# ericyinyzy/VQAttack

Measured on AMD Instinct MI355X. Metric: adversarial_vqa_examples_per_sec, higher is better.
Workload: dtype f32; 1 GPU; vlmo_base VQAttack image PGD (BASELINE configs[1]): batch 64 per GPU, 40 PGD steps, 384x384 images, questions of 6..14 real tokens ([CLS] + n words + [SEP], n ~ U{4..12} seeded) padded to 40 (the all-padding columns are not run through the encoder), eps 0.125 step 0.01 L-inf clip [-1,1], random start, sanity_checks on, black-box scoring + ASR gather; batch_per_gpu=64, pgd_steps=40, image_size=384, text_len=40, substitutable_words=0

## Files before the change

### include/vqattack_hip.h

```cpp
#ifndef VQATTACK_HIP_H
#define VQATTACK_HIP_H

#include <stddef.h>
#include <stdint.h>

#ifdef __cplusplus
extern "C" {
#endif

typedef void* vqa_stream_t;

#define VQA_OK 0
#define VQA_ERR_NULL (-1)
#define VQA_ERR_SHAPE (-2)
#define VQA_ERR_ALIGN (-3)

#define VQA_CLIP 1u
#define VQA_CHECK_RANGE 2u
#define VQA_FLAG_RANGE 1
#define VQA_FLAG_BAD_LABEL 2
#define VQA_FLAG_DEGENERATE 4

int vqa_abi_version(void);
const char* vqa_error_string(int code);
// ... 40 lines not shown

int vqa_l1_fgm(const float* x, const float* g, const float* amax, const float* ties, float* out, int batch,
               size_t n_per_sample, float eps_iter, float cmin, float cmax, unsigned mode, int* flag,
               vqa_stream_t stream);

int vqa_scale_per_sample(const float* t, const float* stat, const float* stat2, float* out, int batch,
                         size_t n_per_sample, float eps, int kind, int* flag, vqa_stream_t stream);

int vqa_neg_cos_partials(void);
int vqa_neg_cos_rows(const float* a, const float* b, float* ga, float* partial, const uint8_t* row_mask,
                     long mask_period, long rows0, long rows1, int D, long a_stride0, long a_stride1,
                     long b_stride0, long b_stride1, long g_stride0, long g_stride1, float gscale,
                     float cos_eps, float* loss_out, int accumulate, vqa_stream_t stream);

int vqa_neg_cos_max_layers(void);
int vqa_neg_cos_rows_multi(const float* const* a, const float* const* b, float* const* ga, int n_layers,
                           float* partial, const uint8_t* row_mask, long mask_period, long rows0, long rows1, int D,
                           long a_stride0, long a_stride1, long b_stride0, long b_stride1, long g_stride0,
                           long g_stride1, float gscale, float cos_eps, float* loss_out, int accumulate,
                           vqa_stream_t stream);

int vqa_sum_partials(const float* partial, int count, float* dst, int accumulate, float scale,
                     vqa_stream_t stream);

int vqa_ce_max_label_sets(void);
long vqa_ce_scratch_floats(int K, long groups);
int vqa_ce_rows(const float* logits, long row_stride, const int64_t* labels, int K, long rows, int V,
                long ignore_index, long rows_per_group, float* scratch, float* grad, float* row_loss, float gscale,
                float* loss_out, int accumulate, int* flag, unsigned char* row_state, vqa_stream_t stream);

int vqa_gather_rows(const float* src, const int64_t* idx, float* dst, int B, int L, int K, int D,
                    vqa_stream_t stream);

int vqa_cand_dir_sim(const float* word, const float* pos, const float* type, const float* gamma,
                     const float* beta, float ln_eps, const float* e_ori, const float* grad,
                     const int32_t* cand, float* out, int n_cand, int L, int K, int D, vqa_stream_t stream);

int vqa_embed_tokens(const float* word, const float* pos, const float* type, const float* gamma, const float* beta,
                     float ln_eps, const int32_t* triples, int n, float* dst, int D, vqa_stream_t stream);

int vqa_greedy_accept(const int32_t* cand, const int32_t* order, const int32_t* seg, int B, int L,
                      const int64_t* ori_ids, int64_t* cur_ids, int32_t* new_id, int32_t* acc_rank, const float* table,
                      int V, int E, float threshold, vqa_stream_t stream);

int vqa_attn_fwd(const float* q, const float* k, const float* v, const float* bias, float* o, float* lse, float* scores,
                 int B, int H, int Sq, int Sk, const long* strides, const long* bias_strides, float scale,
                 const int* key_hole, int nsplit, float* split_ws, vqa_stream_t stream);
long vqa_attn_scores_floats(int B, int H, int Sq, int Sk);
long vqa_attn_split_ws_floats(int B, int H, int Sq, int Sk, int nsplit);

int vqa_attn_bwd(const float* q, const float* k, const float* v, const float* bias, const float* o, const float* go,
                 const float* lse, const float* scores, float* delta, float* dq, float* dk, float* dv, float* ds_ws, int B,
                 int H, int Sq, int Sk, const long* strides, const long* bias_strides, const long* grad_strides,
                 float scale, int nsplit, float* split_ws, vqa_stream_t stream);
long vqa_attn_bwd_ws_floats(int B, int H, int Sq, int Sk);

int vqa_resize_bicubic_h_u8(const uint8_t* src, int h, int w_in, int c, const int32_t* kk, const int32_t* bounds,
                            int ksize, int w_out, uint8_t* dst, vqa_stream_t stream);
int vqa_resize_bicubic_v_normalize(const uint8_t* src, int h_in, int w, int c, const int32_t* kk,
                                   const int32_t* bounds, int ksize, int h_out, float mean, float stdv, float* dst,
                                   vqa_stream_t stream);

int vqa_ln_fwd(const float* x, const float* r0, const float* r1, const float* rscale, float* x_out,
               const float* gamma0, const float* beta0, const float* gamma1, const float* beta1, float* y0, float* y1,
               float* mean, float* rstd, long rows, int D, long period, long split, float eps, vqa_stream_t stream);
int vqa_ln_bwd(const float* dy0, const float* dy1, const float* x, const float* mean, const float* rstd,
               const float* gamma0, const float* gamma1, const float* g_a, const float* g_inj, const float* rscale,
               float* dx, float* dr0, float* dr1, long rows, int D, long period, long split, vqa_stream_t stream);
int vqa_ln_bwd_post(const float* dy_a, const float* dy_b, const float* g_inj, const float* s, const float* rstd,
                    const float* gamma, float* ds, long rows, int D, vqa_stream_t stream);
int vqa_gelu_fwd(const float* h, float* a, size_t n, vqa_stream_t stream);
int vqa_gelu_bwd(const float* h, const float* da, float* dh, size_t n, vqa_stream_t stream);

size_t vqa_gemm_packed_bytes(int K, int N);
int vqa_gemm_pack_b(const float* w, long ldw, int trans, void* packed, int K, int N, vqa_stream_t stream);
int vqa_gemm_bf16x6(const float* A, long lda, const void* packed, const float* bias, float* C, long ldc, long M, int N,
                    int K, vqa_stream_t stream);

#define VQA_GEMM_TILE_256X128 0
#define VQA_GEMM_TILE_128X256 1
int vqa_gemm_bf16x6_tile(const float* A, long lda, const void* packed, const float* bias, float* C, long ldc, long M,
                         int N, int K, int tile, vqa_stream_t stream);

int vqa_gemm_bf16x6_half(const float* A, long lda, const void* packed, const float* bias, float* C, long ldc, long M,
                         int N, int K, vqa_stream_t stream);
int vqa_gemm_bf16x6_tail(const float* A, long lda, const void* packed, const float* bias, float* C, long ldc, long M,
                         int N, int K, int tile, long m_split, vqa_stream_t stream);

size_t vqa_gemm_small_ws_bytes(long M, int N, int ksplit);
int vqa_gemm_bf16x6_small(const float* A, long lda, const void* packed, const float* bias, float* C, long ldc, long M,
                          int N, int K, int ksplit, void* ws, vqa_stream_t stream);

#define VQA_GEMM_EPI_NONE 0
#define VQA_GEMM_EPI_GELU 1
#define VQA_GEMM_EPI_GELU_GRAD 2
int vqa_gemm_bf16x6_epi(const float* A, long lda, const void* packed, const float* bias, float* C, long ldc, long M,
                        int N, int K, int tile, int epilogue, float* aux, long ldaux, vqa_stream_t stream);

#define VQA_GEMM_MAX_GROUPS 4
int vqa_gemm_bf16x6_grouped(const float* const* A, const long* lda, const void* const* packed, const float* const* bias,
                            float* const* C, const long* ldc, float* const* aux, const long* ldaux, const long* M,
                            int n_groups, int N, int K, int epilogue, vqa_stream_t stream);

long vqa_gemm_lse_ws_floats(long M, int N);
int vqa_gemm_bf16x6_lse(const float* A, long lda, const void* packed, const float* bias, long M, int N, int K,
                        int n_valid, const int64_t* targets, long ignore_index, float* ws, float* row_loss, float* lse,
                        int* flag, int tile, vqa_stream_t stream);

#ifdef __cplusplus
}
#endif
#endif
```

### vqattack_amd/_hip.py

```python
import ctypes
import os
import threading

import torch

_HERE = os.path.dirname(os.path.abspath(__file__))
LIB_PATH = os.path.join(_HERE, "lib", "libvqattack_hip.so")
TUNING_LIB_PATH = os.path.join(_HERE, "lib", "libvqattack_hip_tuning.so")

VQA_CLIP = 1
VQA_CHECK_RANGE = 2
VQA_FLAG_RANGE = 1
VQA_FLAG_BAD_LABEL = 2
VQA_FLAG_DEGENERATE = 4
ABI_VERSION = 4

_c_float_p = ctypes.c_void_p
_sz = ctypes.c_size_t
_f = ctypes.c_float
_i = ctypes.c_int
_u = ctypes.c_uint
_l = ctypes.c_long
_p = ctypes.c_void_p

SIGNATURES = {
    "vqa_abi_version": (_i, []),
    "vqa_error_string": (ctypes.c_char_p, [_i]),
    "vqa_linf_init": (_i, [_p, _p, _p, _sz, _f, _f, _f, _u, _p, _p]),
    "vqa_linf_fgm": (_i, [_p, _p, _p, _sz, _f, _f, _f, _u, _p, _p]),
    "vqa_linf_step": (_i, [_p, _p, _p, _p, _sz, _f, _f, _f, _f, _u, _p, _p]),
    "vqa_linf_project": (_i, [_p, _p, _p, _sz, _f, _f, _f, _u, _p]),
    "vqa_clip_eta_linf": (_i, [_p, _p, _sz, _f, _p]),
    "vqa_optimize_linear_linf": (_i, [_p, _p, _sz, _f, _p]),
    "vqa_zero_out_clipped_grads": (_i, [_p, _p, _p, _sz, _f, _f, _p]),
    "vqa_reduce_ws_bytes": (_sz, [_i, _sz]),
    "vqa_sumsq_per_sample": (_i, [_p, _p, _p, _i, _sz, _p, _p]),
    "vqa_absmax_ties_per_sample": (_i, [_p, _p, _p, _i, _sz, _p, _p]),
    "vqa_l2_fgm": (_i, [_p, _p, _p, _p, _i, _sz, _f, _f, _f, _u, _p, _p]),
    "vqa_l2_project": (_i, [_p, _p, _p, _p, _i, _sz, _f, _f, _f, _u, _p]),
    "vqa_l1_fgm": (_i, [_p, _p, _p, _p, _p, _i, _sz, _f, _f, _f, _u, _p, _p]),
    "vqa_scale_per_sample": (_i, [_p, _p, _p, _p, _i, _sz, _f, _i, _p, _p]),
    "vqa_neg_cos_partials": (_i, []),
    "vqa_neg_cos_rows": (_i, [_p, _p, _p, _p, _p, _l, _l, _l, _i, _l, _l, _l, _l, _l, _l, _f, _f, _p, _i, _p]),
    "vqa_neg_cos_max_layers": (_i, []),
    "vqa_neg_cos_rows_multi": (_i, [_p, _p, _p, _i, _p, _p, _l, _l, _l, _i, _l, _l, _l, _l, _l, _l, _f, _f, _p, _i, _p]),
    "vqa_sum_partials": (_i, [_p, _i, _p, _i, _f, _p]),
    "vqa_ce_max_label_sets": (_i, []),
    "vqa_ce_scratch_floats": (_l, [_i, _l]),
    "vqa_ce_rows": (_i, [_p, _l, _p, _i, _l, _i, _l, _l, _p, _p, _p, _f, _p, _i, _p, _p, _p]),
    "vqa_gather_rows": (_i, [_p, _p, _p, _i, _i, _i, _i, _p]),
    "vqa_cand_dir_sim": (_i, [_p, _p, _p, _p, _p, _f, _p, _p, _p, _p, _i, _i, _i, _i, _p]),
    "vqa_embed_tokens": (_i, [_p, _p, _p, _p, _p, _f, _p, _i, _p, _i, _p]),
    "vqa_greedy_accept": (_i, [_p, _p, _p, _i, _i, _p, _p, _p, _p, _p, _i, _i, _f, _p]),
    "vqa_attn_fwd": (_i, [_p, _p, _p, _p, _p, _p, _p, _i, _i, _i, _i, _p, _p, _f, _p, _i, _p, _p]),
    "vqa_attn_split_ws_floats": (_l, [_i, _i, _i, _i, _i]),
    "vqa_attn_scores_floats": (_l, [_i, _i, _i, _i]),
    "vqa_attn_bwd": (_i, [_p, _p, _p, _p, _p, _p, _p, _p, _p, _p, _p, _p, _p, _i, _i, _i, _i, _p, _p, _p, _f, _i, _p, _p]),
    "vqa_attn_bwd_ws_floats": (_l, [_i, _i, _i, _i]),
    "vqa_ln_fwd": (_i, [_p] * 13 + [_l, _i, _l, _l, _f, _p]),
    "vqa_ln_bwd": (_i, [_p] * 13 + [_l, _i, _l, _l, _p]),
    "vqa_ln_bwd_post": (_i, [_p] * 7 + [_l, _i, _p]),
    "vqa_gelu_fwd": (_i, [_p, _p, _sz, _p]),
    "vqa_gelu_bwd": (_i, [_p, _p, _p, _sz, _p]),
    "vqa_resize_bicubic_h_u8": (_i, [_p, _i, _i, _i, _p, _p, _i, _i, _p, _p]),
    "vqa_resize_bicubic_v_normalize": (_i, [_p, _i, _i, _i, _p, _p, _i, _i, _f, _f, _p, _p]),
    "vqa_gemm_packed_bytes": (_sz, [_i, _i]),
    "vqa_gemm_pack_b": (_i, [_p, _l, _i, _p, _i, _i, _p]),
    "vqa_gemm_bf16x6": (_i, [_p, _l, _p, _p, _p, _l, _l, _i, _i, _p]),
    "vqa_gemm_bf16x6_tile": (_i, [_p, _l, _p, _p, _p, _l, _l, _i, _i, _i, _p]),
    "vqa_gemm_bf16x6_half": (_i, [_p, _l, _p, _p, _p, _l, _l, _i, _i, _p]),
    "vqa_gemm_bf16x6_tail": (_i, [_p, _l, _p, _p, _p, _l, _l, _i, _i, _i, _l, _p]),
    "vqa_gemm_small_ws_bytes": (_sz, [_l, _i, _i]),
    "vqa_gemm_bf16x6_small": (_i, [_p, _l, _p, _p, _p, _l, _l, _i, _i, _i, _p, _p]),
    "vqa_gemm_bf16x6_epi": (_i, [_p, _l, _p, _p, _p, _l, _l, _i, _i, _i, _i, _p, _l, _p]),
    "vqa_gemm_bf16x6_grouped": (_i, [_p, _p, _p, _p, _p, _p, _p, _p, _p, _i, _i, _i, _i, _p]),
    "vqa_gemm_lse_ws_floats": (_l, [_l, _i]),
    "vqa_gemm_bf16x6_lse": (_i, [_p, _l, _p, _p, _l, _i, _i, _i, _p, _l, _p, _p, _p, _p, _i, _p]),
}

_lib = None
_lock = threading.Lock()


class HipExtensionError(RuntimeError):
    pass


def load_library(path=None):
    tuning = os.environ.get("VQA_TUNING_LIB", "") not in ("", "0")
    if path is None:
        path = TUNING_LIB_PATH if tuning else LIB_PATH
    if not os.path.exists(path):
        raise HipExtensionError(
            "HIP kernel library not found at {} -- build it with `python -m vqattack_amd.build` "
            "(or __graft_entry__.build()); vqattack_amd has no CPU or eager fallback".format(path))
    if tuning and path == TUNING_LIB_PATH:
        from . import build as _build
        if _build._stale(path):
            raise HipExtensionError("{} is older than vqattack_amd/csrc: rebuild it with `python -m vqattack_amd.build "
                                    "--tuning`".format(path))
    lib = ctypes.CDLL(path)
    for name, (res, args) in SIGNATURES.items():
        fn = getattr(lib, name)
        fn.restype = res
        fn.argtypes = args
    if lib.vqa_abi_version() != ABI_VERSION:
        raise HipExtensionError("{} implements C ABI version {}, this package binds version {}: rebuild it with "
                                "`python -m vqattack_amd.build --force`".format(path, lib.vqa_abi_version(), ABI_VERSION))
    options = [item for item in os.environ.get("VQA_OPTIONS", "").split(",") if item]
    if options:
        if not hasattr(lib, "vqa_set_option"):
            raise HipExtensionError("VQA_OPTIONS needs the tuning build: `python -m vqattack_amd.build --tuning` and "
                                    "VQA_TUNING_LIB=1 ({} has no vqa_set_option)".format(path))
        lib.vqa_set_option.restype, lib.vqa_set_option.argtypes = _i, [_i, _i]
        for item in options:
            opt, val = item.split("=")
            if lib.vqa_set_option(int(opt), int(val)) != 0:
                raise HipExtensionError("bad VQA_OPTIONS entry '{}'".format(item))
    return lib


def lib():
    global _lib
    if _lib is None:
        with _lock:
            if _lib is None:
                _lib = load_library()
    return _lib


def set_option(option, value):
    handle = lib()
    if not hasattr(handle, "vqa_set_option"):
        return False
    handle.vqa_set_option.restype, handle.vqa_set_option.argtypes = _i, [_i, _i]
    if handle.vqa_set_option(int(option), int(value)) != 0:
        raise HipExtensionError("vqa_set_option({}, {}) rejected".format(option, value))
    return True


def check(code, what):
    if code != 0:
        msg = lib().vqa_error_string(code)
        raise HipExtensionError("{} failed: {} ({})".format(what, msg.decode() if msg else "?", code))


def stream_for(t):
    return ctypes.c_void_p(torch.cuda.current_stream(t.device).cuda_stream)


def dev_f32(t, name, contiguous=True):
    if not isinstance(t, torch.Tensor):
# ... 21 lines not shown
```

### vqattack_amd/csrc/gemm.hip

```cpp
#include "common.hpp"
#include "gelu.hpp"

namespace vqa {

typedef __bf16 bf16x8 __attribute__((ext_vector_type(8)));
typedef __bf16 bf16x2 __attribute__((ext_vector_type(2)));
typedef float f32x4 __attribute__((ext_vector_type(4)));

constexpr int kGemmBM = 256, kGemmBN = 128, kGemmBK = 32;
constexpr int kGemmThreads = 512;
constexpr int kGemmMT = kGemmBM / 16, kGemmNT = kGemmBN / 16;
constexpr int kTileBytes = 64 * 16;
constexpr int kGemmABytes = kGemmMT * 3 * kTileBytes;
constexpr int kGemmBBytes = kGemmNT * 3 * kTileBytes;
constexpr int kGemmStage = kGemmABytes + kGemmBBytes;
constexpr int kGemmBPieces = kGemmBBytes / 16 / kGemmThreads;
constexpr int kWideLoadPair = 12;

__device__ __forceinline__ void split2(f32x2 a, bf16x2& h0, bf16x2& h1, bf16x2& h2) {
  h0 = __builtin_convertvector(a, bf16x2);
  f32x2 r = a - __builtin_convertvector(h0, f32x2);
  r.x = __builtin_isfinite(r.x) ? r.x : 0.0f;
  r.y = __builtin_isfinite(r.y) ? r.y : 0.0f;
  h1 = __builtin_convertvector(r, bf16x2);
// ... 692 lines not shown
  long r = m0 + wave * 16 + (lane & 15);
  r = r < g.M ? r : g.M - 1;
  const float* arow = g.A + r * g.lda + 8 * (lane >> 4);
  const bf16x8* bsrc = g.B + static_cast<size_t>(nb) * kWideNT * 3 * 64;
  const size_t bstep = static_cast<size_t>(nt16) * 3 * 64;

  f32x4 ra[2];
  auto load = [&](int kt) {
    ra[0] = *reinterpret_cast<const f32x4*>(arow + kt * kGemmBK);
    ra[1] = *reinterpret_cast<const f32x4*>(arow + kt * kGemmBK + 4);
  };
  char* const bwave = smem + kWideABytes + wave_u * kTileBytes;
  auto load_b = [&](int kt, int s, int p) {
    stage_b16(bsrc + kt * bstep + p * kGemmThreads + tid, bwave + s * kWideStage + p * kGemmThreads * 16);
  };
  auto store = [&](int s) {
    char* base = smem + s * kWideStage;
    bf16x8 p0, p1, p2;
    split8(ra[0], ra[1], p0, p1, p2);
    bf16x8* dst = reinterpret_cast<bf16x8*>(base) + wave * 3 * 64 + lane;
    dst[0] = p0;
    dst[64] = p1;
    dst[128] = p2;
  };

  f32x4 acc[4][4];
#pragma unroll
  for (int i = 0; i < 4; ++i)
#pragma unroll
    for (int j = 0; j < 4; ++j) acc[i][j] = f32x4{0.0f, 0.0f, 0.0f, 0.0f};

  load(0);
#pragma unroll
  for (int p = 0; p < kWideBPieces; ++p) load_b(0, 0, p);
  store(0);
  stage_b_wait();
  __syncthreads();
  for (int kt = 0; kt < nk; ++kt) {
    const int cur = kt & 1;
    const int nxt = kt + 1 < nk ? kt + 1 : kt;
    load(nxt);
    const bf16x8* sa = reinterpret_cast<const bf16x8*>(smem + cur * kWideStage) + wm * 4 * 3 * 64 + lane;
    const bf16x8* sb = reinterpret_cast<const bf16x8*>(smem + cur * kWideStage + kWideABytes) + wn * 4 * 3 * 64 + lane;
    bf16x8 fa[3][4], fb[3][4];
#pragma unroll
    for (int i = 0; i < 4; ++i)
#pragma unroll
      for (int p = 0; p < 3; ++p) {
        fa[p][i] = sa[(i * 3 + p) * 64];
        fb[p][i] = sb[(i * 3 + p) * 64];
      }
    constexpr int kPa[6] = {2, 1, 0, 1, 0, 0}, kPb[6] = {0, 1, 2, 0, 1, 0};
#pragma unroll
    for (int t = 0; t < 6; ++t) {
      if (t == 3) store(cur ^ 1);
#pragma unroll
      for (int i = 0; i < 4; ++i)
#pragma unroll
        for (int j = 0; j < 4; ++j) {
          acc[i][j] = __builtin_amdgcn_mfma_f32_16x16x32_bf16(fb[kPb[t]][j], fa[kPa[t]][i], acc[i][j], 0, 0, 0);
          if ((t * 16 + i * 4 + j + 1) % kWideLoadPair == 0 && (t * 16 + i * 4 + j + 1) / kWideLoadPair <= kWideBPieces / 2) {
            const int pair = (t * 16 + i * 4 + j + 1) / kWideLoadPair - 1;
            load_b(nxt, cur ^ 1, 2 * pair);
            load_b(nxt, cur ^ 1, 2 * pair + 1);
          }
        }
    }
#pragma unroll
    for (int n = 0; n < (2 + kWideBPieces) / 2; ++n) {
      __builtin_amdgcn_sched_group_barrier(0x020, 2, 0);
      __builtin_amdgcn_sched_group_barrier(0x008, kWideLoadPair, 0);
    }
    stage_b_wait();
    __syncthreads();
  }

  if constexpr (EPI == VQA_GEMM_EPI_NONE) {
    gemm_store(acc, g, m0 + wm * 64, n0 + wn * 64, lane);
  } else {
    gemm_epilogue<EPI>(acc, g, m0 + wm * 64, n0 + wn * 64, lane);
  }
}

constexpr int kSmallBM = 64;
constexpr int kSmallThreads = 256;
constexpr int kSmallMT = kSmallBM / 16;
constexpr int kSmallABytes = kSmallMT * 3 * kTileBytes;
constexpr int kSmallStage = kSmallABytes + kGemmBBytes;
constexpr int kSmallBPieces = kGemmBBytes / 16 / kSmallThreads;
constexpr int kGemmMaxKSplit = 16;

__global__ __launch_bounds__(kSmallThreads) void gemm_bf16x6_small_kernel(GemmArgs g, float* __restrict__ ws, int ksplit) {
  __shared__ __attribute__((aligned(16))) char smem[2 * kSmallStage];
  const int tid = threadIdx.x, lane = tid & 63, wave = tid >> 6;
  const int wm = wave >> 1, wn = wave & 1;
  const int ntb = g.N / kGemmBN;
  const int mtb = static_cast<int>((g.M + kSmallBM - 1) / kSmallBM);
  const int tiles = mtb * ntb;
  const int nwg = tiles * ksplit, orig = blockIdx.x, xcd = orig & 7, q = nwg >> 3, rem = nwg & 7;
  const int wg = (xcd < rem ? xcd * (q + 1) : rem * (q + 1) + (xcd - rem) * q) + (orig >> 3);
  const int part = wg / tiles, tile = wg - part * tiles;
  const int mb = tile / ntb, nb = tile - mb * ntb;
  const long m0 = static_cast<long>(mb) * kSmallBM;
  const int n0 = nb * kGemmBN;
  const int nk = g.K / kGemmBK;
  const int k0 = part * nk / ksplit, k1 = (part + 1) * nk / ksplit;
  const int nt16 = g.N / 16;

  long r = m0 + wave * 16 + (lane & 15);
  r = r < g.M ? r : g.M - 1;
  const float* arow = g.A + r * g.lda + 8 * (lane >> 4);
  const bf16x8* bsrc = g.B + static_cast<size_t>(nb) * kGemmNT * 3 * 64;
  const size_t bstep = static_cast<size_t>(nt16) * 3 * 64;

  f32x4 ra[2];
  bf16x8 rb[kSmallBPieces];
  auto load = [&](int kt) {
    ra[0] = *reinterpret_cast<const f32x4*>(arow + kt * kGemmBK);
    ra[1] = *reinterpret_cast<const f32x4*>(arow + kt * kGemmBK + 4);
#pragma unroll
    for (int p = 0; p < kSmallBPieces; ++p) rb[p] = bsrc[kt * bstep + p * kSmallThreads + tid];
  };
  auto store = [&](int s) {
    char* base = smem + s * kSmallStage;
    bf16x8 p0, p1, p2;
    split8(ra[0], ra[1], p0, p1, p2);
    bf16x8* dst = reinterpret_cast<bf16x8*>(base) + wave * 3 * 64 + lane;
    dst[0] = p0;
    dst[64] = p1;
    dst[128] = p2;
    bf16x8* bdst = reinterpret_cast<bf16x8*>(base + kSmallABytes);
#pragma unroll
    for (int p = 0; p < kSmallBPieces; ++p) bdst[p * kSmallThreads + tid] = rb[p];
  };

  f32x4 acc[2][4];
#pragma unroll
  for (int i = 0; i < 2; ++i)
#pragma unroll
    for (int j = 0; j < 4; ++j) acc[i][j] = f32x4{0.0f, 0.0f, 0.0f, 0.0f};

  load(k0);
  store(0);
  __syncthreads();
  for (int kt = k0; kt < k1; ++kt) {
    const int cur = (kt - k0) & 1;
    load(kt + 1 < k1 ? kt + 1 : kt);
    __builtin_amdgcn_sched_barrier(0);
    const bf16x8* sa = reinterpret_cast<const bf16x8*>(smem + cur * kSmallStage) + wm * 2 * 3 * 64 + lane;
    const bf16x8* sb = reinterpret_cast<const bf16x8*>(smem + cur * kSmallStage + kSmallABytes) + wn * 4 * 3 * 64 + lane;
    bf16x8 fa[3][2], fb[3][4];
#pragma unroll
    for (int p = 0; p < 3; ++p) {
#pragma unroll
      for (int i = 0; i < 2; ++i) fa[p][i] = sa[(i * 3 + p) * 64];
#pragma unroll
      for (int j = 0; j < 4; ++j) fb[p][j] = sb[(j * 3 + p) * 64];
    }
    constexpr int kPa[6] = {2, 1, 0, 1, 0, 0}, kPb[6] = {0, 1, 2, 0, 1, 0};
#pragma unroll
    for (int t = 0; t < 6; ++t) {
      if (t == 3) store(cur ^ 1);
#pragma unroll
      for (int i = 0; i < 2; ++i)
#pragma unroll
        for (int j = 0; j < 4; ++j)
// ... 206 lines not shown
      }
    }
    row_loss[row] = loss;
  }
}

__global__ __launch_bounds__(kBlock) void gemm_pack_b_kernel(const float* __restrict__ w, long ldw, int trans,
                                                             bf16x8* __restrict__ out, int K, int N) {
  const long total = static_cast<long>(K / 32) * (N / 16) * 64;
  for (long idx = static_cast<long>(blockIdx.x) * blockDim.x + threadIdx.x; idx < total;
       idx += static_cast<long>(gridDim.x) * blockDim.x) {
    const int l = static_cast<int>(idx & 63);
    const long tile = idx >> 6;
    const int nt = static_cast<int>(tile % (N / 16)), kt = static_cast<int>(tile / (N / 16));
    const int n = nt * 16 + (l & 15), k = kt * 32 + 8 * (l >> 4);
    float v[8];
#pragma unroll
    for (int e = 0; e < 8; ++e) v[e] = trans ? w[static_cast<long>(n) * ldw + k + e] : w[static_cast<long>(k + e) * ldw + n];
    bf16x8 p0, p1, p2;
    split8(f32x4{v[0], v[1], v[2], v[3]}, f32x4{v[4], v[5], v[6], v[7]}, p0, p1, p2);
    out[(tile * 3 + 0) * 64 + l] = p0;
    out[(tile * 3 + 1) * 64 + l] = p1;
    out[(tile * 3 + 2) * 64 + l] = p2;
  }
}

}

using namespace vqa;

static int gemm_vec_ok(const float* C, long ldc, const float* bias, const float* aux = nullptr, long ldaux = 0) {
  return aligned16(C) && ldc % 4 == 0 && (!bias || aligned16(bias)) && (!aux || (aligned16(aux) && ldaux % 4 == 0));
}

extern "C" {

size_t vqa_gemm_packed_bytes(int K, int N) {
  if (K <= 0 || N <= 0 || K % kGemmBK || N % kGemmBN) return 0;
  return static_cast<size_t>(K) * N * 3 * sizeof(__bf16);
}

int vqa_gemm_pack_b(const float* w, long ldw, int trans, void* packed, int K, int N, vqa_stream_t stream) {
  clear_stale_error();
  if (!w || !packed) return VQA_ERR_NULL;
  if (K <= 0 || N <= 0 || K % kGemmBK || N % kGemmBN || (trans != 0 && trans != 1)) return VQA_ERR_SHAPE;
  if (ldw < (trans ? K : N)) return VQA_ERR_SHAPE;
  if (!aligned4(w) || !aligned16(packed)) return VQA_ERR_ALIGN;
  const long work = static_cast<long>(K / 32) * (N / 16) * 64;
  gemm_pack_b_kernel<<<blocks_for(work, kBlock), kBlock, 0, static_cast<hipStream_t>(stream)>>>(
      w, ldw, trans, static_cast<bf16x8*>(packed), K, N);
  return launch_status();
}

int vqa_gemm_bf16x6(const float* A, long lda, const void* packed, const float* bias, float* C, long ldc, long M, int N,
                    int K, vqa_stream_t stream) {
  clear_stale_error();
  if (!A || !packed || !C) return VQA_ERR_NULL;
  if (M < 0 || N <= 0 || K <= 0 || K % kGemmBK || N % kGemmBN || lda < K || lda % 4 || ldc < N) return VQA_ERR_SHAPE;
  if ((M + kGemmBM - 1) / kGemmBM * (N / kGemmBN) > 0x7fffffffL) return VQA_ERR_SHAPE;
  if (!aligned16(A) || !aligned16(packed) || !aligned4(C) || (bias && !aligned4(bias))) return VQA_ERR_ALIGN;
  if (M == 0) return VQA_OK;
  GemmArgs g{A, static_cast<const bf16x8*>(packed), bias, C, lda, ldc, M, N, K, gemm_vec_ok(C, ldc, bias)};
  const int grid = static_cast<int>((M + kGemmBM - 1) / kGemmBM * (N / kGemmBN));
  gemm_bf16x6_kernel<<<grid, kGemmThreads, 0, static_cast<hipStream_t>(stream)>>>(g);
  return launch_status();
}

int vqa_gemm_bf16x6_tile(const float* A, long lda, const void* packed, const float* bias, float* C, long ldc, long M,
                         int N, int K, int tile, vqa_stream_t stream) {
  if (tile != VQA_GEMM_TILE_256X128 && tile != VQA_GEMM_TILE_128X256) {
    clear_stale_error();
    return VQA_ERR_SHAPE;
  }
  if (tile == VQA_GEMM_TILE_256X128 || N <= 0 || N % kWideBN) return vqa_gemm_bf16x6(A, lda, packed, bias, C, ldc, M, N, K, stream);
  clear_stale_error();
  if (!A || !packed || !C) return VQA_ERR_NULL;
  if (M < 0 || K <= 0 || K % kGemmBK || lda < K || lda % 4 || ldc < N) return VQA_ERR_SHAPE;
  if ((M + kWideBM - 1) / kWideBM * (N / kWideBN) > 0x7fffffffL) return VQA_ERR_SHAPE;
  if (!aligned16(A) || !aligned16(packed) || !aligned4(C) || (bias && !aligned4(bias))) return VQA_ERR_ALIGN;
  if (M == 0) return VQA_OK;
  GemmArgs g{A, static_cast<const bf16x8*>(packed), bias, C, lda, ldc, M, N, K, gemm_vec_ok(C, ldc, bias)};
  const int grid = static_cast<int>((M + kWideBM - 1) / kWideBM * (N / kWideBN));
  gemm_bf16x6_wide_kernel<<<grid, kGemmThreads, 0, static_cast<hipStream_t>(stream)>>>(g);
  return launch_status();
}

int vqa_gemm_bf16x6_half(const float* A, long lda, const void* packed, const float* bias, float* C, long ldc, long M,
                         int N, int K, vqa_stream_t stream) {
  clear_stale_error();
  if (!A || !packed || !C) return VQA_ERR_NULL;
  if (M < 0 || N <= 0 || K <= 0 || K % kGemmBK || N % kGemmBN || lda < K || lda % 4 || ldc < N) return VQA_ERR_SHAPE;
  if ((M + kHalfBM - 1) / kHalfBM * (N / kGemmBN) > 0x7fffffffL) return VQA_ERR_SHAPE;
  if (!aligned16(A) || !aligned16(packed) || !aligned4(C) || (bias && !aligned4(bias))) return VQA_ERR_ALIGN;
  if (M == 0) return VQA_OK;
  GemmArgs g{A, static_cast<const bf16x8*>(packed), bias, C, lda, ldc, M, N, K, gemm_vec_ok(C, ldc, bias)};
  const int grid = static_cast<int>((M + kHalfBM - 1) / kHalfBM * (N / kGemmBN));
  gemm_bf16x6_half_kernel<<<grid, kGemmThreads, 0, static_cast<hipStream_t>(stream)>>>(g);
  return launch_status();
}

int vqa_gemm_bf16x6_tail(const float* A, long lda, const void* packed, const float* bias, float* C, long ldc, long M,
                         int N, int K, int tile, long m_split, vqa_stream_t stream) {
  clear_stale_error();
  if (tile != VQA_GEMM_TILE_256X128 && tile != VQA_GEMM_TILE_128X256) return VQA_ERR_SHAPE;
  if (!A || !packed || !C) return VQA_ERR_NULL;
  if (M < 0 || m_split < 0 || m_split > M) return VQA_ERR_SHAPE;
  if (m_split == M) return vqa_gemm_bf16x6_tile(A, lda, packed, bias, C, ldc, M, N, K, tile, stream);
  if (m_split == 0) return vqa_gemm_bf16x6_half(A, lda, packed, bias, C, ldc, M, N, K, stream);
  if (N <= 0 || K <= 0 || K % kGemmBK || N % kGemmBN || lda < K || lda % 4 || ldc < N) return VQA_ERR_SHAPE;
  if (!aligned16(A) || !aligned16(packed) || !aligned4(C) || (bias && !aligned4(bias))) return VQA_ERR_ALIGN;
  const int rc = vqa_gemm_bf16x6_tile(A, lda, packed, bias, C, ldc, m_split, N, K, tile, stream);
  if (rc != VQA_OK) return rc;
  return vqa_gemm_bf16x6_half(A + m_split * lda, lda, packed, bias, C + m_split * ldc, ldc, M - m_split, N, K, stream);
}

int vqa_gemm_bf16x6_epi(const float* A, long lda, const void* packed, const float* bias, float* C, long ldc, long M,
                        int N, int K, int tile, int epilogue, float* aux, long ldaux, vqa_stream_t stream) {
  if (epilogue == VQA_GEMM_EPI_NONE) return vqa_gemm_bf16x6_tile(A, lda, packed, bias, C, ldc, M, N, K, tile, stream);
  clear_stale_error();
  if (tile != VQA_GEMM_TILE_256X128 && tile != VQA_GEMM_TILE_128X256) return VQA_ERR_SHAPE;
  if (epilogue != VQA_GEMM_EPI_GELU && epilogue != VQA_GEMM_EPI_GELU_GRAD) return VQA_ERR_SHAPE;
  if (!A || !packed || !C || (epilogue == VQA_GEMM_EPI_GELU_GRAD && !aux)) return VQA_ERR_NULL;
  if (M < 0 || N <= 0 || K <= 0 || K % kGemmBK || N % kGemmBN || lda < K || lda % 4 || ldc < N) return VQA_ERR_SHAPE;
  if (aux && ldaux < N) return VQA_ERR_SHAPE;
  const bool wide = tile == VQA_GEMM_TILE_128X256 && N % kWideBN == 0;
  const long grid = wide ? (M + kWideBM - 1) / kWideBM * (N / kWideBN) : (M + kGemmBM - 1) / kGemmBM * (N / kGemmBN);
  if (grid > 0x7fffffffL) return VQA_ERR_SHAPE;
  if (!aligned16(A) || !aligned16(packed) || !aligned4(C) || (bias && !aligned4(bias)) || (aux && !aligned4(aux)))
    return VQA_ERR_ALIGN;
  if (aux && (aux == C || aux == A)) return VQA_ERR_SHAPE;
  if (M == 0) return VQA_OK;
  GemmEpiArgs e{{A, static_cast<const bf16x8*>(packed), bias, C, lda, ldc, M, N, K, gemm_vec_ok(C, ldc, bias, aux, ldaux)},
                aux, ldaux};
  hipStream_t st = static_cast<hipStream_t>(stream);
  const int nwg = static_cast<int>(grid);
  if (wide) {
    if (epilogue == VQA_GEMM_EPI_GELU) gemm_bf16x6_wide_epi_kernel<VQA_GEMM_EPI_GELU><<<nwg, kGemmThreads, 0, st>>>(e);
    else gemm_bf16x6_wide_epi_kernel<VQA_GEMM_EPI_GELU_GRAD><<<nwg, kGemmThreads, 0, st>>>(e);
  } else {
    if (epilogue == VQA_GEMM_EPI_GELU) gemm_bf16x6_epi_kernel<VQA_GEMM_EPI_GELU><<<nwg, kGemmThreads, 0, st>>>(e);
    else gemm_bf16x6_epi_kernel<VQA_GEMM_EPI_GELU_GRAD><<<nwg, kGemmThreads, 0, st>>>(e);
  }
  return launch_status();
}

int vqa_gemm_bf16x6_grouped(const float* const* A, const long* lda, const void* const* packed, const float* const* bias,
                            float* const* C, const long* ldc, float* const* aux, const long* ldaux, const long* M,
                            int n_groups, int N, int K, int epilogue, vqa_stream_t stream) {
  clear_stale_error();
  if (n_groups < 1 || n_groups > VQA_GEMM_MAX_GROUPS) return VQA_ERR_SHAPE;
  if (epilogue != VQA_GEMM_EPI_NONE && epilogue != VQA_GEMM_EPI_GELU && epilogue != VQA_GEMM_EPI_GELU_GRAD) return VQA_ERR_SHAPE;
  if (!A || !lda || !packed || !C || !ldc || !M || (aux && !ldaux)) return VQA_ERR_NULL;
  if (N <= 0 || K <= 0 || K % kGemmBK || N % kWideBN) return VQA_ERR_SHAPE;
  GemmGroupedArgs ga{};
  ga.N = N, ga.K = K, ga.vec = 1;
  long blocks = 0;
  for (int i = 0; i < n_groups; ++i) {
    if (M[i] < 0) return VQA_ERR_SHAPE;
    ga.start[i] = static_cast<int>(blocks);
    if (M[i] == 0) continue;
    const float* b = bias ? bias[i] : nullptr;
    float* x = (aux && epilogue != VQA_GEMM_EPI_NONE) ? aux[i] : nullptr;
    const long ldx = x ? ldaux[i] : 0;
    if (!A[i] || !packed[i] || !C[i] || (epilogue == VQA_GEMM_EPI_GELU_GRAD && !x)) return VQA_ERR_NULL;
    if (lda[i] < K || lda[i] % 4 || ldc[i] < N || (x && ldx < N)) return VQA_ERR_SHAPE;
    blocks += (M[i] + kWideBM - 1) / kWideBM;
// ... 80 lines not shown
```

### vqattack_amd/ops.py

```python
import contextlib
import ctypes

import torch

from . import _hip
from ._hip import VQA_CHECK_RANGE, VQA_CLIP, check, dev_f32, lib, ptr, same_device, stream_for

_INF = float("inf")


@contextlib.contextmanager
def _on(t):
    if t.device.index is not None and t.device.index != torch.cuda.current_device():
        with torch.cuda.device(t.device):
            yield
    else:
        yield


def _clip_args(clip_min, clip_max):
    if clip_min is None and clip_max is None:
        return 0, -_INF, _INF
    return VQA_CLIP, (-_INF if clip_min is None else float(clip_min)), (_INF if clip_max is None else float(clip_max))

# ... 617 lines not shown

    def __init__(self, data, K, N, n_valid=None):
        self.data, self.K, self.N = data, K, N
        self.n_valid = N if n_valid is None else int(n_valid)
        if not 0 < self.n_valid <= N:
            raise ValueError("n_valid must be in (0, {}], got {}".format(N, n_valid))


def gemm_shape_ok(N, K):
    return N > 0 and K > 0 and N % 128 == 0 and K % 32 == 0


def gemm_workgroups(M, N):
    return -(-M // 256) * (N // 128)


def gemm_pack(w, trans):
    dev_f32(w, "w")
    if w.dim() != 2:
        raise ValueError("w must be 2-D, got shape {}".format(tuple(w.shape)))
    K, N = (w.shape[1], w.shape[0]) if trans else (w.shape[0], w.shape[1])
    nbytes = lib().vqa_gemm_packed_bytes(K, N)
    if nbytes == 0:
        raise ValueError("vqa_gemm_pack_b does not cover K={}, N={}".format(K, N))
    data = torch.empty(nbytes, dtype=torch.uint8, device=w.device)
    with _on(w):
        check(lib().vqa_gemm_pack_b(_p(w), w.shape[1], int(bool(trans)), _p(data), K, N, stream_for(w)), "vqa_gemm_pack_b")
    return PackedWeight(data, K, N)


VOCAB_PAD = 256


def gemm_pack_vocab(w):
    dev_f32(w, "w")
    if w.dim() != 2:
        raise ValueError("w must be 2-D, got shape {}".format(tuple(w.shape)))
    V, K = w.shape
    Vp = -(-V // VOCAB_PAD) * VOCAB_PAD
    if Vp != V:
        padded = torch.zeros(Vp, K, dtype=torch.float32, device=w.device)
        padded[:V] = w
        w = padded
    packed = gemm_pack(w.contiguous(), trans=True)
    return PackedWeight(packed.data, packed.K, packed.N, V)


GEMM_TILES = {"large": 0, "wide": 1}


GEMM_EPILOGUES = {"gelu": 1, "gelu_grad": 2}


def gemm_tail_plan(M, N, tile, cus):
    if tile not in GEMM_TILES:
        raise ValueError("tile must be one of {}, got {!r}".format(sorted(GEMM_TILES), tile))
    M, N, cus = int(M), int(N), int(cus)
    bm, bn = (128, 256) if tile == "wide" and N % 256 == 0 else (256, 128)
    ntb = N // bn
    nwg = -(-M // bm) * ntb
    full = (nwg // cus) * cus if cus > 0 else 0
    if full == 0 or nwg == full:
        return M
    m_split = (full // ntb) * bm
    tail = -(-(M - m_split) // 128) * (N // 128)
    return m_split if tail <= cus else M


def gemm(a, packed, bias=None, out=None, tile=None, epilogue=None, aux=None, m_split=None):
    if epilogue is not None and epilogue not in GEMM_EPILOGUES:
        raise ValueError("epilogue must be None or one of {}, got {!r}".format(sorted(GEMM_EPILOGUES), epilogue))
    if epilogue is None and aux is not None:
        raise ValueError("aux goes with an epilogue")
    if epilogue == "gelu_grad" and aux is None:
        raise ValueError("epilogue 'gelu_grad' needs aux = the pre-activation h")
    if aux is not None:
        if aux is out:
            raise ValueError("aux must not be out")
        M = a.shape[0]
        if not isinstance(aux, torch.Tensor) or tuple(aux.shape) != (M, packed.N) or aux.stride(1) != 1 or \
                (M > 1 and aux.stride(0) < packed.N):
            raise ValueError("aux must be a ({}, {}) tensor with unit column stride, got {}".format(
                M, packed.N, (tuple(aux.shape), aux.stride()) if isinstance(aux, torch.Tensor) else type(aux)))
    if tile is None:
        from .whitebox import _fused
        tile = _fused.gemm_tile(a.shape[0], packed.N, packed.K)
    if tile not in GEMM_TILES:
        raise ValueError("tile must be one of {}, got {!r}".format(sorted(GEMM_TILES), tile))
    if m_split is not None:
        if epilogue is not None:
            raise ValueError("m_split does not go with an epilogue")
        if isinstance(m_split, bool) or not isinstance(m_split, int) or not 0 <= m_split <= a.shape[0]:
            raise ValueError("m_split must be an integer in [0, {}], got {!r}".format(a.shape[0], m_split))
        return _gemm_rows(a, packed, bias, out, tile, m_split)
    if epilogue is not None:
        return _gemm_epilogue(a, packed, bias, out, tile, epilogue, aux)
    return _gemm_tiled(a, packed, bias, out, tile)


def gemm_half(a, packed, bias=None, out=None):
    return _gemm_rows(a, packed, bias, out, None, 0)


def _gemm_tiled(a, packed, bias, out, tile):
    return _gemm_rows(a, packed, bias, out, tile, None)


TAIL_CALLS = [0]


def _gemm_rows(a, packed, bias, out, tile, m_split):
    dev_f32(a, "a", contiguous=False)
    if a.dim() != 2 or a.shape[1] != packed.K or a.stride(1) != 1 or a.stride(0) % 4:
        raise ValueError("a must be (M, {}) with unit column stride and a row stride % 4 == 0, got shape {} strides {}"
                         .format(packed.K, tuple(a.shape), a.stride()))
    M = a.shape[0]
    if out is None:
        out = torch.empty(M, packed.N, dtype=torch.float32, device=a.device)
    dev_f32(out, "out")
    if tuple(out.shape) != (M, packed.N):
        raise ValueError("out must be ({}, {}), got {}".format(M, packed.N, tuple(out.shape)))
    if bias is not None:
        dev_f32(bias, "bias"), _rows_ok("bias", bias, packed.N)
    same_device(a, packed.data, bias, out)
    if M:
        planned = tile is not None and m_split is None
        if planned:
            from .whitebox import _fused
            m_split = _fused.gemm_tail_split(M, packed.N, packed.K, tile, a.device)
        with _on(a):
            if tile is None:
                check(lib().vqa_gemm_bf16x6_half(_p(a), a.stride(0), _p(packed.data), ptr(bias), _p(out), packed.N, M,
                                                 packed.N, packed.K, stream_for(a)), "vqa_gemm_bf16x6_half")
            elif planned and m_split >= M:
                check(lib().vqa_gemm_bf16x6_tile(_p(a), a.stride(0), _p(packed.data), ptr(bias), _p(out), packed.N, M,
                                                 packed.N, packed.K, GEMM_TILES[tile], stream_for(a)), "vqa_gemm_bf16x6_tile")
            else:
                TAIL_CALLS[0] += 1
                check(lib().vqa_gemm_bf16x6_tail(_p(a), a.stride(0), _p(packed.data), ptr(bias), _p(out), packed.N, M,
                                                 packed.N, packed.K, GEMM_TILES[tile], m_split, stream_for(a)),
                      "vqa_gemm_bf16x6_tail")
    return out


def _gemm_epilogue(a, packed, bias, out, tile, epilogue, aux):
    dev_f32(a, "a", contiguous=False)
    if a.dim() != 2 or a.shape[1] != packed.K or a.stride(1) != 1 or a.stride(0) % 4:
        raise ValueError("a must be (M, {}) with unit column stride and a row stride % 4 == 0, got shape {} strides {}"
                         .format(packed.K, tuple(a.shape), a.stride()))
    M, N = a.shape[0], packed.N
    if out is None:
        out = torch.empty(M, N, dtype=torch.float32, device=a.device)
    dev_f32(out, "out", contiguous=False)
    if tuple(out.shape) != (M, N) or out.stride(1) != 1 or (M > 1 and out.stride(0) < N):
        raise ValueError("out must be ({}, {}) with unit column stride, got {} strides {}".format(
            M, N, tuple(out.shape), out.stride()))
    if bias is not None:
        dev_f32(bias, "bias"), _rows_ok("bias", bias, N)
    if aux is not None:
        dev_f32(aux, "aux", contiguous=False)
        if aux.data_ptr() in (out.data_ptr(), a.data_ptr()):
            raise ValueError("aux must not alias out or a")
    same_device(a, packed.data, bias, out, aux)
    if M:
        with _on(a):
            check(lib().vqa_gemm_bf16x6_epi(_p(a), a.stride(0), _p(packed.data), ptr(bias), _p(out), max(out.stride(0), N), M,
                                            N, packed.K, GEMM_TILES[tile], GEMM_EPILOGUES[epilogue], ptr(aux),
                                            max(aux.stride(0), N) if aux is not None else 0, stream_for(a)),
                  "vqa_gemm_bf16x6_epi")
    return out


GEMM_MAX_GROUPS = 4


def gemm_grouped_blocks(Ms, N):
    N = int(N)
    if N <= 0 or N % 256:
        raise ValueError("the grouped launch runs 128 x 256 tiles: N % 256 == 0, got {}".format(N))
    starts = [0]
    for m in Ms:
        m = int(m)
        if m < 0:
            raise ValueError("row counts must be >= 0, got {}".format(tuple(Ms)))
        starts.append(starts[-1] + -(-m // 128))
    return tuple(starts), starts[-1] * (N // 256)

# ... 143 lines not shown
```

### vqattack_amd/whitebox/_fused.py

```python
import os

import torch

from .. import attention as _attn
from .. import ops

MIN_WORKGROUPS = 192

SMALL_POLICY = {}

_WIDE_ROWS = (35264, 37824)
WIDE_POLICY = {(768, 768): _WIDE_ROWS, (3072, 768): _WIDE_ROWS, (768, 3072): _WIDE_ROWS}

EPILOGUE_POLICY = {"gelu": {}, "gelu_grad": {(3072, 768): _WIDE_ROWS}}

TAIL_POLICY = {}

GROUPED_POLICY = {}

_CUS = {}


def _mode():
    mode = os.environ.get("VQA_GEMM", "")
    return mode if mode in ("library", "large", "wide", "small") else ""


def gemm_tile(rows, n, k):
    mode = _mode()
    if mode == "wide":
        return "wide"
    lo, hi = WIDE_POLICY.get((n, k), (1, 0))
    return "wide" if mode == "" and lo <= rows <= hi else "large"


def _kernel_gemms():
    return _mode() != "library"


def gemm_tail_split(rows, n, k, tile, device):
    switch = os.environ.get("VQA_GEMM_TAIL", "")
    if switch == "0":
        return rows
    if switch != "1":
        lo, hi = TAIL_POLICY.get((n, k), (1, 0))
        if switch != "" or not lo <= rows <= hi:
            return rows
    pinned = os.environ.get("VQA_GEMM_TAIL_CUS")
    if pinned:
        cus = int(pinned)
    else:
        dev = torch.device(device).index or 0
        if dev not in _CUS:
            _CUS[dev] = torch.cuda.get_device_properties(dev).multi_processor_count
        cus = _CUS[dev]
    return ops.gemm_tail_plan(rows, n, tile, cus)


def _small_gemm(rows, n, k):
    mode = _mode()
    if mode == "small":
        return True
    lo, hi = SMALL_POLICY.get((n, k), (1, 0))
    return mode == "" and lo <= rows <= hi


def gelu_epilogue(rows, n, k, epilogue="gelu"):
    if not _kernel_gemms() or ops.gemm_workgroups(rows, n) < MIN_WORKGROUPS:
        return False
    switch = os.environ.get("VQA_GEMM_EPILOGUE", "")
    if switch in ("0", "1"):
        return switch == "1"
    lo, hi = EPILOGUE_POLICY[epilogue].get((n, k), (1, 0))
    return lo <= rows <= hi


def _pack(w):
    if not _kernel_gemms() or not (ops.gemm_shape_ok(w.shape[0], w.shape[1]) and ops.gemm_shape_ok(w.shape[1], w.shape[0])):
        return (None, None)
    return (ops.gemm_pack(w, trans=True), ops.gemm_pack(w, trans=False))


def _linear(a, w, bias, packed):
    pk = packed[0]
    if pk is not None and _kernel_gemms():
        if ops.gemm_workgroups(a.shape[0], pk.N) >= MIN_WORKGROUPS:
            return ops.gemm(a, pk, bias)
        if a.shape[0] and _small_gemm(a.shape[0], pk.N, pk.K):
            return ops.gemm_small(a, pk, bias, ksplit=ops.gemm_small_plan(a.shape[0], pk.N, pk.K))
    return torch.addmm(bias, a, w.t())


def _linear_grad(g, w, packed):
    pk = packed[1]
    if pk is not None and _kernel_gemms():
        if ops.gemm_workgroups(g.shape[0], pk.N) >= MIN_WORKGROUPS:
            return ops.gemm(g, pk)
        if g.shape[0] and _small_gemm(g.shape[0], pk.N, pk.K):
            return ops.gemm_small(g, pk, ksplit=ops.gemm_small_plan(g.shape[0], pk.N, pk.K))
    return torch.mm(g, w)


def _linear_gelu(a, w, bias, packed, save):
    pk = packed[0]
    if pk is not None and gelu_epilogue(a.shape[0], pk.N, pk.K):
        h = torch.empty(a.shape[0], pk.N, dtype=torch.float32, device=a.device) if save else None
        return h, ops.gemm(a, pk, bias, epilogue="gelu", aux=h)
    h = _linear(a, w, bias, packed)
    return (h if save else None), ops.gelu_fwd(h)


def _linear_grad_gelu(g, w, packed, h):
    pk = packed[1]
    if pk is not None and gelu_epilogue(g.shape[0], pk.N, pk.K, "gelu_grad"):
        return ops.gemm(g, pk, epilogue="gelu_grad", aux=h)
    return ops.gelu_bwd(h, _linear_grad(g, w, packed))


def gemm_grouped_pair(rows, n, k):
    big = max(rows)
    if not _kernel_gemms() or n % 256 or min(rows) <= 0 or ops.gemm_workgroups(big, n) < MIN_WORKGROUPS:
        return False
    switch = os.environ.get("VQA_GEMM_GROUPED", "")
    if switch in ("0", "1"):
        return switch == "1"
    lo, hi = GROUPED_POLICY.get((n, k), (1, 0))
    return lo <= big <= hi


def _pair_order(rows, pks):
    if len(pks) != 2 or pks[0] is None or pks[1] is None or (pks[0].N, pks[0].K) != (pks[1].N, pks[1].K):
        return None
    if not gemm_grouped_pair(rows, pks[0].N, pks[0].K):
        return None
    return (0, 1) if rows[0] >= rows[1] else (1, 0)


def _pair_call(order, xs, pks, biases=None, epilogue=None, aux=None):
    def pick(ts):
# ... 585 lines not shown
```

Measured before the change: 15.98 examples/s.

## Add persistent 128x256 GEMM kernel for QKV-shaped projections

Adds a persistent bf16x6 GEMM kernel that launches one workgroup per CU and walks a contiguous run of 128x256 output tiles per workgroup, grouped by XCD. It prefetches the next tile's first A/B slices during the last k-step of the current tile. A policy routes the QKV-shaped GEMMs (N,K = 2304/768 and 768/2304) in a given row range to it when the caller named no tile. The aim is to remove wave-quantization tail and launch/ramp costs of the one-shot tiled grid, at the cost of more complex scheduling and possible load imbalance.

```diff
diff --git a/include/vqattack_hip.h b/include/vqattack_hip.h
--- a/include/vqattack_hip.h
+++ b/include/vqattack_hip.h
@@ -146,6 +146,9 @@
 int vqa_gemm_bf16x6_tile(const float* A, long lda, const void* packed, const float* bias, float* C, long ldc, long M,
                          int N, int K, int tile, vqa_stream_t stream);
 
+int vqa_gemm_bf16x6_persistent(const float* A, long lda, const void* packed, const float* bias, float* C, long ldc, long M,
+                               int N, int K, int workgroups, vqa_stream_t stream);
+
 int vqa_gemm_bf16x6_half(const float* A, long lda, const void* packed, const float* bias, float* C, long ldc, long M,
                          int N, int K, vqa_stream_t stream);
 int vqa_gemm_bf16x6_tail(const float* A, long lda, const void* packed, const float* bias, float* C, long ldc, long M,
diff --git a/vqattack_amd/_hip.py b/vqattack_amd/_hip.py
--- a/vqattack_amd/_hip.py
+++ b/vqattack_amd/_hip.py
@@ -68,6 +68,7 @@
     "vqa_gemm_pack_b": (_i, [_p, _l, _i, _p, _i, _i, _p]),
     "vqa_gemm_bf16x6": (_i, [_p, _l, _p, _p, _p, _l, _l, _i, _i, _p]),
     "vqa_gemm_bf16x6_tile": (_i, [_p, _l, _p, _p, _p, _l, _l, _i, _i, _i, _p]),
+    "vqa_gemm_bf16x6_persistent": (_i, [_p, _l, _p, _p, _p, _l, _l, _i, _i, _i, _p]),
     "vqa_gemm_bf16x6_half": (_i, [_p, _l, _p, _p, _p, _l, _l, _i, _i, _p]),
     "vqa_gemm_bf16x6_tail": (_i, [_p, _l, _p, _p, _p, _l, _l, _i, _i, _i, _l, _p]),
     "vqa_gemm_small_ws_bytes": (_sz, [_l, _i, _i]),
diff --git a/vqattack_amd/csrc/gemm.hip b/vqattack_amd/csrc/gemm.hip
--- a/vqattack_amd/csrc/gemm.hip
+++ b/vqattack_amd/csrc/gemm.hip
@@ -798,6 +798,128 @@
   }
 }
 
+__global__ __launch_bounds__(kGemmThreads) void gemm_bf16x6_persistent_kernel(GemmArgs g, int ntiles) {
+  __shared__ __attribute__((aligned(16))) char smem[2 * kWideStage];
+  const int tid = threadIdx.x, lane = tid & 63, wave = tid >> 6;
+  const int wave_u = __builtin_amdgcn_readfirstlane(wave);
+  const int wm = wave >> 2, wn = wave & 3;
+  const int ntb = g.N / kWideBN;
+  const int nk = g.K / kGemmBK;
+  const int nt16 = g.N / 16;
+  const int nwg = gridDim.x, orig = blockIdx.x, xcd = orig & 7, q = nwg >> 3, rem = nwg & 7;
+  const int wx = q + (xcd < rem ? 1 : 0);
+  const int pos = xcd < rem ? xcd * (q + 1) : rem * (q + 1) + (xcd - rem) * q;
+  const int run0 = static_cast<int>(static_cast<long>(ntiles) * pos / nwg);
+  const int run1 = static_cast<int>(static_cast<long>(ntiles) * (pos + wx) / nwg);
+  int tile = run0 + (orig >> 3);
+  if (tile >= run1) return;
+
+  const size_t bstep = static_cast<size_t>(nt16) * 3 * 64;
+  auto locate = [&](int t, long& m0, int& n0, const float*& arow, const bf16x8*& bsrc) {
+    const int mb = t / ntb, nb = t - mb * ntb;
+    m0 = static_cast<long>(mb) * kWideBM;
+    n0 = nb * kWideBN;
+    long r = m0 + wave * 16 + (lane & 15);
+    r = r < g.M ? r : g.M - 1;
+    arow = g.A + r * g.lda + 8 * (lane >> 4);
+    bsrc = g.B + static_cast<size_t>(nb) * kWideNT * 3 * 64;
+  };
+  long m0;
+  int n0;
+  const float* arow;
+  const bf16x8* bsrc;
+  locate(tile, m0, n0, arow, bsrc);
+
+  f32x4 ra[2];
+  auto load = [&](const float* src) {
+    ra[0] = *reinterpret_cast<const f32x4*>(src);
+    ra[1] = *reinterpret_cast<const f32x4*>(src + 4);
+  };
+  char* const bwave = smem + kWideABytes + wave_u * kTileBytes;
+  auto load_b = [&](const bf16x8* src, int s, int p) {
+    stage_b16(src + p * kGemmThreads + tid, bwave + s * kWideStage + p * kGemmThreads * 16);
+  };
+  auto store = [&](int s) {
+    char* base = smem + s * kWideStage;
+    bf16x8 p0, p1, p2;
+    split8(ra[0], ra[1], p0, p1, p2);
+    bf16x8* dst = reinterpret_cast<bf16x8*>(base) + wave * 3 * 64 + lane;
+    dst[0] = p0;
+    dst[64] = p1;
+    dst[128] = p2;
+  };
+
+  f32x4 acc[4][4];
+#pragma unroll
+  for (int i = 0; i < 4; ++i)
+#pragma unroll
+    for (int j = 0; j < 4; ++j) acc[i][j] = f32x4{0.0f, 0.0f, 0.0f, 0.0f};
+
+  load(arow);
+#pragma unroll
+  for (int p = 0; p < kWideBPieces; ++p) load_b(bsrc, 0, p);
+  store(0);
+  stage_b_wait();
+  __syncthreads();
+  int cur = 0;
+  for (;;) {
+    const int tnext = tile + wx;
+    const bool more = tnext < run1;
+    long m0n = m0;
+    int n0n = n0;
+    const float* arow_n = arow + (nk - 1) * kGemmBK;
+    const bf16x8* bsrc_n = bsrc + (nk - 1) * bstep;
+    if (more) locate(tnext, m0n, n0n, arow_n, bsrc_n);
+    auto step = [&](const float* anxt, const bf16x8* bnxt) {
+      load(anxt);
+      const bf16x8* sa = reinterpret_cast<const bf16x8*>(smem + cur * kWideStage) + wm * 4 * 3 * 64 + lane;
+      const bf16x8* sb = reinterpret_cast<const bf16x8*>(smem + cur * kWideStage + kWideABytes) + wn * 4 * 3 * 64 + lane;
+      bf16x8 fa[3][4], fb[3][4];
+#pragma unroll
+      for (int i = 0; i < 4; ++i)
+#pragma unroll
+        for (int p = 0; p < 3; ++p) {
+          fa[p][i] = sa[(i * 3 + p) * 64];
+          fb[p][i] = sb[(i * 3 + p) * 64];
+        }
+      constexpr int kPa[6] = {2, 1, 0, 1, 0, 0}, kPb[6] = {0, 1, 2, 0, 1, 0};
+#pragma unroll
+      for (int t = 0; t < 6; ++t) {
+        if (t == 3) store(cur ^ 1);
+#pragma unroll
+        for (int i = 0; i < 4; ++i)
+#pragma unroll
+          for (int j = 0; j < 4; ++j) {
+            acc[i][j] = __builtin_amdgcn_mfma_f32_16x16x32_bf16(fb[kPb[t]][j], fa[kPa[t]][i], acc[i][j], 0, 0, 0);
+            if ((t * 16 + i * 4 + j + 1) % kWideLoadPair == 0 && (t * 16 + i * 4 + j + 1) / kWideLoadPair <= kWideBPieces / 2) {
+              const int pair = (t * 16 + i * 4 + j + 1) / kWideLoadPair - 1;
+              load_b(bnxt, cur ^ 1, 2 * pair);
+              load_b(bnxt, cur ^ 1, 2 * pair + 1);
+            }
+          }
+      }
+#pragma unroll
+      for (int n = 0; n < (2 + kWideBPieces) / 2; ++n) {
+        __builtin_amdgcn_sched_group_barrier(0x020, 2, 0);
+        __builtin_amdgcn_sched_group_barrier(0x008, kWideLoadPair, 0);
+      }
+      stage_b_wait();
+      __syncthreads();
+      cur ^= 1;
+    };
+    for (int kt = 0; kt + 1 < nk; ++kt) step(arow + (kt + 1) * kGemmBK, bsrc + (kt + 1) * bstep);
+    step(arow_n, bsrc_n);
+
+    gemm_store(acc, g, m0 + wm * 64, n0 + wn * 64, lane);
+    if (!more) break;
+#pragma unroll
+    for (int i = 0; i < 4; ++i)
+#pragma unroll
+      for (int j = 0; j < 4; ++j) acc[i][j] = f32x4{0.0f, 0.0f, 0.0f, 0.0f};
+    tile = tnext, m0 = m0n, n0 = n0n, arow = arow_n, bsrc = bsrc_n;
+  }
+}
+
 constexpr int kSmallBM = 64;
 constexpr int kSmallThreads = 256;
 constexpr int kSmallMT = kSmallBM / 16;
@@ -1170,6 +1292,21 @@
   GemmArgs g{A, static_cast<const bf16x8*>(packed), bias, C, lda, ldc, M, N, K, gemm_vec_ok(C, ldc, bias)};
   const int grid = static_cast<int>((M + kWideBM - 1) / kWideBM * (N / kWideBN));
   gemm_bf16x6_wide_kernel<<<grid, kGemmThreads, 0, static_cast<hipStream_t>(stream)>>>(g);
+  return launch_status();
+}
+
+int vqa_gemm_bf16x6_persistent(const float* A, long lda, const void* packed, const float* bias, float* C, long ldc, long M,
+                               int N, int K, int workgroups, vqa_stream_t stream) {
+  clear_stale_error();
+  if (!A || !packed || !C) return VQA_ERR_NULL;
+  if (M < 0 || N <= 0 || K <= 0 || K % kGemmBK || N % kWideBN || lda < K || lda % 4 || ldc < N || workgroups < 1) return VQA_ERR_SHAPE;
+  if ((M + kWideBM - 1) / kWideBM * (N / kWideBN) > 0x7fffffffL) return VQA_ERR_SHAPE;
+  if (!aligned16(A) || !aligned16(packed) || !aligned4(C) || (bias && !aligned4(bias))) return VQA_ERR_ALIGN;
+  if (M == 0) return VQA_OK;
+  GemmArgs g{A, static_cast<const bf16x8*>(packed), bias, C, lda, ldc, M, N, K, gemm_vec_ok(C, ldc, bias)};
+  const int ntiles = static_cast<int>((M + kWideBM - 1) / kWideBM * (N / kWideBN));
+  const int grid = workgroups < ntiles ? workgroups : ntiles;
+  gemm_bf16x6_persistent_kernel<<<grid, kGemmThreads, 0, static_cast<hipStream_t>(stream)>>>(g, ntiles);
   return launch_status();
 }
 
diff --git a/vqattack_amd/ops.py b/vqattack_amd/ops.py
--- a/vqattack_amd/ops.py
+++ b/vqattack_amd/ops.py
@@ -723,11 +723,15 @@
                 (M > 1 and aux.stride(0) < packed.N):
             raise ValueError("aux must be a ({}, {}) tensor with unit column stride, got {}".format(
                 M, packed.N, (tuple(aux.shape), aux.stride()) if isinstance(aux, torch.Tensor) else type(aux)))
+    if tile == "persistent":
+        if epilogue is not None or m_split is not None:
+            raise ValueError("tile 'persistent' goes with neither an epilogue nor m_split")
+        return gemm_persistent(a, packed, bias, out)
     if tile is None:
         from .whitebox import _fused
-        tile = _fused.gemm_tile(a.shape[0], packed.N, packed.K)
+        tile = _PolicyTile(_fused.gemm_tile(a.shape[0], packed.N, packed.K))
     if tile not in GEMM_TILES:
-        raise ValueError("tile must be one of {}, got {!r}".format(sorted(GEMM_TILES), tile))
+        raise ValueError("tile must be one of {}, got {!r}".format(sorted(GEMM_TILES) + ["persistent"], tile))
     if m_split is not None:
         if epilogue is not None:
             raise ValueError("m_split does not go with an epilogue")
@@ -739,11 +743,51 @@
     return _gemm_tiled(a, packed, bias, out, tile)
 
 
+class _PolicyTile(str):
+    """A tile name that ``gemm`` took from ``_fused.gemm_tile`` because its caller named none: equal to the plain name
+    everywhere, and the mark by which ``_gemm_tiled`` knows that ``_fused.gemm_persistent`` may replace the launch."""
+
+
+def gemm_persistent(a, packed, bias=None, out=None, workgroups=None):
+    dev_f32(a, "a", contiguous=False)
+    if a.dim() != 2 or a.shape[1] != packed.K or a.stride(1) != 1 or a.stride(0) % 4:
+        raise ValueError("a must be (M, {}) with unit column stride and a row stride % 4 == 0, got shape {} strides {}"
+                         .format(packed.K, tuple(a.shape), a.stride()))
+    M, N = a.shape[0], packed.N
+    if N % 256:
+        raise ValueError("the persistent launch runs 128 x 256 tiles: N % 256 == 0, got N = {}".format(N))
+    if workgroups is not None and (isinstance(workgroups, bool) or not isinstance(workgroups, int) or workgroups < 1):
+        raise ValueError("workgroups must be None or an integer >= 1, got {!r}".format(workgroups))
+    if out is None:
+        out = torch.empty(M, N, dtype=torch.float32, device=a.device)
+    dev_f32(out, "out", contiguous=False)
+    if tuple(out.shape) != (M, N) or out.stride(1) != 1 or (M > 1 and out.stride(0) < N):
+        raise ValueError("out must be ({}, {}) with unit column stride, got {} strides {}".format(
+            M, N, tuple(out.shape), out.stride()))
+    if bias is not None:
+        dev_f32(bias, "bias"), _rows_ok("bias", bias, N)
+    same_device(a, packed.data, bias, out)
+    if M:
+        if workgroups is None:
+            from .whitebox import _fused
+            workgroups = _fused.device_cus(a.device)
+        with _on(a):
+            check(lib().vqa_gemm_bf16x6_persistent(_p(a), a.stride(0), _p(packed.data), ptr(bias), _p(out),
+                                                   max(out.stride(0), N), M, N, packed.K, min(workgroups, 0x7fffffff),
+                                                   stream_for(a)), "vqa_gemm_bf16x6_persistent")
+    return out
+
+
 def gemm_half(a, packed, bias=None, out=None):
     return _gemm_rows(a, packed, bias, out, None, 0)
 
 
 def _gemm_tiled(a, packed, bias, out, tile):
+    M = a.shape[0]
+    if isinstance(tile, _PolicyTile) and packed.N % 256 == 0 and M:
+        from .whitebox import _fused
+        if _fused.gemm_persistent(M, packed.N, packed.K) and _fused.gemm_tail_split(M, packed.N, packed.K, tile, a.device) >= M:
+            return gemm_persistent(a, packed, bias, out)
     return _gemm_rows(a, packed, bias, out, tile, None)
 
 
diff --git a/vqattack_amd/whitebox/_fused.py b/vqattack_amd/whitebox/_fused.py
--- a/vqattack_amd/whitebox/_fused.py
+++ b/vqattack_amd/whitebox/_fused.py
@@ -17,6 +17,9 @@
 TAIL_POLICY = {}
 
 GROUPED_POLICY = {}
+
+_QKV_ROWS = (37312, 39488)
+PERSISTENT_POLICY = {(2304, 768): _QKV_ROWS, (768, 2304): _QKV_ROWS}
 
 _CUS = {}
 
@@ -34,8 +37,25 @@
     return "wide" if mode == "" and lo <= rows <= hi else "large"
 
 
+def gemm_persistent(rows, n, k):
+    if n % 256 or _mode() != "":
+        return False
+    switch = os.environ.get("VQA_GEMM_PERSISTENT", "")
+    if switch in ("0", "1"):
+        return switch == "1"
+    lo, hi = PERSISTENT_POLICY.get((n, k), (1, 0))
+    return lo <= rows <= hi
+
+
 def _kernel_gemms():
     return _mode() != "library"
+
+
+def device_cus(device):
+    dev = torch.device(device).index or 0
+    if dev not in _CUS:
+        _CUS[dev] = torch.cuda.get_device_properties(dev).multi_processor_count
+    return _CUS[dev]
 
 
 def gemm_tail_split(rows, n, k, tile, device):
@@ -47,14 +67,7 @@
         if switch != "" or not lo <= rows <= hi:
             return rows
     pinned = os.environ.get("VQA_GEMM_TAIL_CUS")
-    if pinned:
-        cus = int(pinned)
-    else:
-        dev = torch.device(device).index or 0
-        if dev not in _CUS:
-            _CUS[dev] = torch.cuda.get_device_properties(dev).multi_processor_count
-        cus = _CUS[dev]
-    return ops.gemm_tail_plan(rows, n, tile, cus)
+    return ops.gemm_tail_plan(rows, n, tile, int(pinned) if pinned else device_cus(device))
 
 
 def _small_gemm(rows, n, k):
```

After: 16.24 examples/s, median of 6. 1.02x the previous value.
